# chanchanchan97/ICAFusion

Measured on AMD Instinct MI355X. Metric: RGB/IR image-pairs/sec (two-stream forward + NMS), higher is better.
Workload: dtype bf16

## Files before the change

### icafusion_amd/csrc/conv_common.h

```cpp
#pragma once
#include "icaf_common.h"

namespace icaf {

struct ConvP {
    const void* x; const void* w; const float* bias; void* y; const void* res;
    long long x_gs, w_gs, bias_gs, y_gs, res_gs;
    int B, H, W, Cin, ldx, Ho, Wo, Cout, ldy, kh, kw, sh, sw, ph, pw, ldr, Kp, act;
    int M, K, nchunks, mtiles, ntiles;
    int vec_y, vec_r;
    unsigned int x_bytes, w_bytes;
    float alpha_acc[2], alpha_res[2];
    const float* pre; int pre_h, pre_w, ldpre, pre_mode;
    const void* w1; const float* bias1;
    long long w1_gs, bias1_gs; int Kp1; unsigned int w1_bytes;
    const void* w2; const float* bias2; void* y2;
    long long w2_gs, bias2_gs, y2_gs; int Kp2, Cout2, ldy2, vec_y2, keep1; unsigned int w2_bytes;
    const void* x2; long long x2_gs; int ldx2;
};

constexpr int ROWB = 64;
constexpr int ROWS = 80;
constexpr int NTHREADS = 256;

int ctile_conv_check(const icaf_conv_args* a, const ConvP& p, int shape);
int launch_ctile(const icaf_conv_args* a, const ConvP& p, int shape, hipStream_t s);
const char* ctile_tag(int shape);
int stream_check(const icaf_conv_args* a, const ConvP& p, int shape);
int launch_stream(const icaf_conv_args* a, const ConvP& p, int shape, hipStream_t s);
const char* stream_tag(int shape);
int wreg_check(const icaf_conv_args* a, const ConvP& p, int shape);
int launch_wreg(const icaf_conv_args* a, const ConvP& p, int shape, hipStream_t s);
const char* wreg_tag(int shape);
int cstream_check(const icaf_conv_args* a, const ConvP& p, int shape);
int launch_cstream(const icaf_conv_args* a, const ConvP& p, int shape, hipStream_t s);
const char* cstream_tag(int shape);
int cwide_check(const icaf_conv_args* a, const ConvP& p, int shape);
int launch_cwide(const icaf_conv_args* a, const ConvP& p, int shape, hipStream_t s);
const char* cwide_tag(int shape);
int launch_bneck(const icaf_conv_args* a, const ConvP& p, int shape, hipStream_t s);

template <int ACT, int DT = ICAF_F32> __device__ __forceinline__ float apply_act(float v) {
    if constexpr (ACT == ICAF_ACT_SILU) return silu_f(v);
    else if constexpr (ACT == ICAF_ACT_GELU) return DT == ICAF_F32 ? gelu_f(v) : gelu_fast_f(v);
    else return v;
}
template <int ACT, int DT = ICAF_F32> __device__ __forceinline__ void apply_act4(const float (&x)[4], float (&y)[4]) {
    if constexpr (ACT == ICAF_ACT_SILU) silu4_f(x, y);
    else {
#pragma unroll
        for (int j = 0; j < 4; ++j) y[j] = apply_act<ACT, DT>(x[j]);
    }
}

__device__ __forceinline__ int xcd_tile(int ntile_total) {
    const int bid = blockIdx.x, q = ntile_total >> 3, r = ntile_total & 7, xcd = bid & 7, idx = bid >> 3;
    return (xcd < r ? xcd * (q + 1) : r * (q + 1) + (xcd - r) * q) + idx;
}

#ifndef ICAF_EPI_FAST
#define ICAF_EPI_FAST 1
#endif
#ifndef ICAF_PRE_WB
#define ICAF_PRE_WB 1
#endif
template <int DT, int ODT, int BM, int BN, int WM, int WN, int ACT, bool PRE, bool SECOND = false, bool WB = false, bool FULLVEC = false, typename RowMap>
__device__ __forceinline__ void epilogue(f32x16 (&acc)[WN / 32][WM / 32], unsigned char* lds, const ConvP& p, int g, RowMap row_to_m, int n0) {
    using E = Elem<DT>;
    using EO = Elem<ODT>;
    constexpr int TM = WM / 32, TN = WN / 32;
    constexpr int WAVES_M = BM / WM;
    constexpr int NT = (BM / WM) * (BN / WN) * 64;
    constexpr int VO = 16 / EO::BYTES;
    constexpr int SO = BN * EO::BYTES + 16;
    const int tid = threadIdx.x, lane = tid & 63, wave = tid >> 6, l31 = lane & 31, hi = lane >> 5;
    const int wm = wave % WAVES_M, wn = wave / WAVES_M;
    const float alpha_acc = SECOND ? 1.0f : p.alpha_acc[g], alpha_res = p.alpha_res[g];
    const float* __restrict__ bias = SECOND ? (p.bias2 ? p.bias2 + g * p.bias2_gs : nullptr) : (p.bias ? p.bias + g * p.bias_gs : nullptr);
    const int Cout = SECOND ? p.Cout2 : p.Cout, ldy = SECOND ? p.ldy2 : p.ldy, vec_y = SECOND ? p.vec_y2 : p.vec_y;
    if constexpr (PRE && ICAF_PRE_WB) {
        constexpr int SOF = BN * 4 + 16;
#pragma unroll
        for (int a = 0; a < TN; ++a) {
            f32x4 bq[4];
#pragma unroll
            for (int q = 0; q < 4; ++q) {
                const int n = n0 + wn * WN + a * 32 + 8 * q + 4 * hi;
                const bool okn = bias && n < Cout;
                const float* bp = okn ? bias + n : (const float*)p.w;
                const f32x4 t = *(const f32x4*)bp;
                bq[q] = okn ? t : f32x4{0.f, 0.f, 0.f, 0.f};
            }
#pragma unroll
            for (int q = 0; q < 4; ++q) {
                const int nl = wn * WN + a * 32 + 8 * q + 4 * hi;
#pragma unroll
                for (int b = 0; b < TM; ++b) {
                    const int ml = wm * WM + b * 32 + l31;
                    f32x4 t;
#pragma unroll
                    for (int j = 0; j < 4; ++j) t[j] = acc[a][b][4 * q + j] + bq[q][j];
                    *(f32x4*)(lds + ml * SOF + nl * 4) = t;
                }
            }
        }
        __syncthreads();
        typename EO::type* __restrict__ yg2 = SECOND ? (typename EO::type*)p.y2 + g * p.y2_gs : (typename EO::type*)p.y + g * p.y_gs;
        const typename E::type* __restrict__ rg2 = (!SECOND && p.res) ? (const typename E::type*)p.res + g * p.res_gs : nullptr;
        constexpr int VPR2 = BN / VO, NVEC2 = BM * VPR2, NIT2 = (NVEC2 + NT - 1) / NT;
        const float sy = (float)p.pre_h / (float)p.Ho, sx = (float)p.pre_w / (float)p.Wo;
#pragma unroll 2
        for (int it = 0; it < NIT2; ++it) {
            const int idx = tid + it * NT;
            if (idx >= NVEC2) break;
            const int row = idx / VPR2, cv = idx - row * VPR2;
            const int m = row_to_m(row), n = n0 + cv * VO;
            if (m < 0 || n >= Cout) continue;
            const float* pt4[4];
            float lx, ly;
            {
#pragma clang fp contract(off)
                const int wo = m % p.Wo, t = m / p.Wo, ho = t % p.Ho, bi = t / p.Ho;
                float fy = ((float)ho + 0.5f) * sy - 0.5f, fx = ((float)wo + 0.5f) * sx - 0.5f;
                fy = fy < 0.0f ? 0.0f : fy;
                fx = fx < 0.0f ? 0.0f : fx;
                int y0 = (int)fy, x0 = (int)fx;
                y0 = y0 < p.pre_h - 1 ? y0 : p.pre_h - 1;
                x0 = x0 < p.pre_w - 1 ? x0 : p.pre_w - 1;
                int y1 = y0 < p.pre_h - 1 ? y0 + 1 : y0, x1 = x0 < p.pre_w - 1 ? x0 + 1 : x0;
                ly = fy - (float)y0;
                lx = fx - (float)x0;
                if (p.pre_mode == 1) {
                    y0 = y1 = (int)((long long)ho * p.pre_h / p.Ho);
                    x0 = x1 = (int)((long long)wo * p.pre_w / p.Wo);
                    ly = lx = 0.0f;
                }
                const float* base = p.pre + (long long)bi * p.pre_h * p.pre_w * p.ldpre + n;
                pt4[0] = base + (long long)(y0 * p.pre_w + x0) * p.ldpre;
                pt4[1] = base + (long long)(y0 * p.pre_w + x1) * p.ldpre;
                pt4[2] = base + (long long)(y1 * p.pre_w + x0) * p.ldpre;
                pt4[3] = base + (long long)(y1 * p.pre_w + x1) * p.ldpre;
            }
            const int nvalid = (Cout - n) < VO ? (Cout - n) : VO;
            float v[VO];
#pragma unroll
            for (int k4 = 0; k4 < VO / 4; ++k4) {
                const f32x4 t = *(const f32x4*)(lds + row * SOF + (cv * VO + 4 * k4) * 4);
                float pv[4] = {0.f, 0.f, 0.f, 0.f};
                if (n + 4 * k4 < Cout) {
                    const f32x4 t00 = *(const f32x4*)(pt4[0] + 4 * k4), t01 = *(const f32x4*)(pt4[1] + 4 * k4);
                    const f32x4 t10 = *(const f32x4*)(pt4[2] + 4 * k4), t11 = *(const f32x4*)(pt4[3] + 4 * k4);
                    {
#pragma clang fp contract(off)
                        const float wx0 = 1.0f - lx, wy0 = 1.0f - ly;
#pragma unroll
                        for (int j = 0; j < 4; ++j) {
                            const float top = t00[j] * wx0 + t01[j] * lx;
                            const float bot = t10[j] * wx0 + t11[j] * lx;
                            pv[j] = top * wy0 + bot * ly;
                        }
                    }
                }
#pragma unroll
                for (int j = 0; j < 4; ++j) v[4 * k4 + j] = apply_act<ACT, DT>(t[j] + pv[j]) * alpha_acc;
            }
            u32x4 o = pack16<ODT>(v);
            typename EO::type* yp = yg2 + (long long)m * ldy + n;
            if (rg2) {
                unpack16<ODT>(o, v);
                const typename E::type* rp = rg2 + (long long)m * p.ldr + n;
                for (int j = 0; j < nvalid; ++j) v[j] = __builtin_fmaf(alpha_res, E::ld(rp + j), v[j]);
                o = pack16<ODT>(v);
            }
            if (vec_y && nvalid == VO) *(u32x4*)yp = o;
            else {
                unpack16<ODT>(o, v);
                for (int j = 0; j < nvalid; ++j) EO::st(yp + j, v[j]);
            }
        }
        return;
    }
    const float* pt[PRE ? TM : 1][4];
    float plx[PRE ? TM : 1], ply[PRE ? TM : 1];
    if constexpr (PRE) {
#pragma clang fp contract(off)
        const float sy = (float)p.pre_h / (float)p.Ho, sx = (float)p.pre_w / (float)p.Wo;
#pragma unroll
        for (int b = 0; b < TM; ++b) {
            const int m = row_to_m(wm * WM + b * 32 + l31);
            const int mm = m < 0 ? 0 : m;
            const int wo = mm % p.Wo, t = mm / p.Wo, ho = t % p.Ho, bi = t / p.Ho;
            float fy = ((float)ho + 0.5f) * sy - 0.5f, fx = ((float)wo + 0.5f) * sx - 0.5f;
            fy = fy < 0.0f ? 0.0f : fy;
            fx = fx < 0.0f ? 0.0f : fx;
            int y0 = (int)fy, x0 = (int)fx;
            y0 = y0 < p.pre_h - 1 ? y0 : p.pre_h - 1;
            x0 = x0 < p.pre_w - 1 ? x0 : p.pre_w - 1;
            int y1 = y0 < p.pre_h - 1 ? y0 + 1 : y0, x1 = x0 < p.pre_w - 1 ? x0 + 1 : x0;
            ply[b] = fy - (float)y0;
            plx[b] = fx - (float)x0;
            if (p.pre_mode == 1) {
                y0 = y1 = (int)((long long)ho * p.pre_h / p.Ho);
                x0 = x1 = (int)((long long)wo * p.pre_w / p.Wo);
                ply[b] = plx[b] = 0.0f;
            }
            const float* base = p.pre + (long long)bi * p.pre_h * p.pre_w * p.ldpre;
            pt[b][0] = base + (long long)(y0 * p.pre_w + x0) * p.ldpre;
            pt[b][1] = base + (long long)(y0 * p.pre_w + x1) * p.ldpre;
            pt[b][2] = base + (long long)(y1 * p.pre_w + x0) * p.ldpre;
            pt[b][3] = base + (long long)(y1 * p.pre_w + x1) * p.ldpre;
        }
    }
#pragma unroll
    for (int a = 0; a < TN; ++a) {
        f32x4 bq[4];
#pragma unroll
        for (int q = 0; q < 4; ++q) {
            const int n = n0 + wn * WN + a * 32 + 8 * q + 4 * hi;
            const bool okn = bias && n < Cout;
            const float* bp = okn ? bias + n : (const float*)p.w;
            const f32x4 t = *(const f32x4*)bp;
            bq[q] = okn ? t : f32x4{0.f, 0.f, 0.f, 0.f};
        }
#pragma unroll
        for (int q = 0; q < 4; ++q) {
            const int nl = wn * WN + a * 32 + 8 * q + 4 * hi;
            const float bv[4] = {bq[q][0], bq[q][1], bq[q][2], bq[q][3]};
#pragma unroll
            for (int b = 0; b < TM; ++b) {
                const int ml = wm * WM + b * 32 + l31;
                float pv[4] = {0.f, 0.f, 0.f, 0.f};
                if constexpr (PRE) if (n0 + nl < Cout) {
                    const f32x4 t00 = *(const f32x4*)(pt[b][0] + n0 + nl), t01 = *(const f32x4*)(pt[b][1] + n0 + nl);
                    const f32x4 t10 = *(const f32x4*)(pt[b][2] + n0 + nl), t11 = *(const f32x4*)(pt[b][3] + n0 + nl);
                    {
#pragma clang fp contract(off)
                        const float wx0 = 1.0f - plx[b], wy0 = 1.0f - ply[b];
#pragma unroll
                        for (int j = 0; j < 4; ++j) {
                            const float top = t00[j] * wx0 + t01[j] * plx[b];
                            const float bot = t10[j] * wx0 + t11[j] * plx[b];
                            pv[j] = top * wy0 + bot * ply[b];
                        }
                    }
                }
                float v[4], xin[4];
#pragma unroll
                for (int j = 0; j < 4; ++j) xin[j] = acc[a][b][4 * q + j] + bv[j] + pv[j];
                apply_act4<ACT, DT>(xin, v);
#pragma unroll
                for (int j = 0; j < 4; ++j) v[j] *= alpha_acc;
                unsigned char* dst = lds + ml * SO + nl * EO::BYTES;
                if constexpr (EO::BYTES == 4) {
                    *(f32x4*)dst = f32x4{v[0], v[1], v[2], v[3]};
                } else {
                    u32x2 pk;
                    if constexpr (ODT == ICAF_BF16) { pk[0] = pack2_bf16(v[0], v[1]); pk[1] = pack2_bf16(v[2], v[3]); }
                    else { pk[0] = pack2_f16(v[0], v[1]); pk[1] = pack2_f16(v[2], v[3]); }
                    *(u32x2*)dst = pk;
                }
            }
        }
    }
    __syncthreads();

    typename EO::type* __restrict__ yg = SECOND ? (typename EO::type*)p.y2 + g * p.y2_gs : (typename EO::type*)p.y + g * p.y_gs;
    const typename E::type* __restrict__ rg = (!SECOND && p.res) ? (const typename E::type*)p.res + g * p.res_gs : nullptr;
    constexpr int VPR = BN / VO;
    constexpr int NVEC = BM * VPR;
    constexpr int NIT = (NVEC + NT - 1) / NT;
    if constexpr (FULLVEC) {
        static_assert(!WB && NVEC % NT == 0 && (VPR & (VPR - 1)) == 0, "whole rounds of power-of-two rows");
#pragma unroll
        for (int it = 0; it < NIT; ++it) {
            const int idx = tid + it * NT, row = idx / VPR, cv = idx & (VPR - 1);
            const int m = row_to_m(row);
            if (m >= 0) *(u32x4*)(yg + (long long)m * ldy + n0 + cv * VO) = *(const u32x4*)(lds + row * SO + cv * 16);
        }
        return;
    }
#if ICAF_EPI_FAST
    if constexpr (VO == E::VEC && NVEC % NT == 0 && (VPR & (VPR - 1)) == 0) {
        if (vec_y && n0 + BN <= Cout && (!rg || p.vec_r)) {
            if (!rg) {
#pragma unroll
                for (int it = 0; it < NIT; ++it) {
                    const int idx = tid + it * NT, row = idx / VPR, cv = idx & (VPR - 1);
                    const int m = row_to_m(row);
                    if (m >= 0) *(u32x4*)(yg + (long long)m * ldy + n0 + cv * VO) = *(const u32x4*)(lds + row * SO + cv * 16);
                }
            } else {
                u32x4 rv[NIT];
#pragma unroll
                for (int it = 0; it < NIT; ++it) {
                    const int idx = tid + it * NT, row = idx / VPR, cv = idx & (VPR - 1);
                    const int m = row_to_m(row);
                    rv[it] = *(const u32x4*)(rg + (long long)(m < 0 ? 0 : m) * p.ldr + n0 + cv * VO);
                }
#pragma unroll
                for (int it = 0; it < NIT; ++it) {
                    const int idx = tid + it * NT, row = idx / VPR, cv = idx & (VPR - 1);
                    const int m = row_to_m(row);
                    if (m < 0) continue;
                    float v[VO], r[VO];
                    unpack16<ODT>(*(const u32x4*)(lds + row * SO + cv * 16), v);
                    unpack16<DT>(rv[it], r);
#pragma unroll
                    for (int j = 0; j < VO; ++j) v[j] = __builtin_fmaf(alpha_res, r[j], v[j]);
                    const u32x4 o = pack16<ODT>(v);
                    if constexpr (WB) *(u32x4*)(lds + row * SO + cv * 16) = o;
                    *(u32x4*)(yg + (long long)m * ldy + n0 + cv * VO) = o;
                }
            }
            return;
        }
#pragma unroll 1
        for (int it = 0; it < NIT; ++it) {
            const int idx = tid + it * NT, row = idx / VPR, cv = idx & (VPR - 1);
            const int m = row_to_m(row), n = n0 + cv * VO;
            if (m < 0 || n >= Cout) continue;
            const u32x4 sv = *(const u32x4*)(lds + row * SO + cv * 16);
// ... 141 lines not shown
```

### icafusion_amd/csrc/detect.hip

```cpp
#pragma clang fp contract(off)
#include "icaf_common.h"
#include "stream_core.h"
#include <cstdlib>

namespace icaf {

struct Anchors { float v[16]; };
int conv_prepare(const icaf_conv_args* a, ConvP& p);

struct DetectDiv { FastDiv no, nx, ny, na; };

template <bool I32>
__global__ __launch_bounds__(256) void detect_decode_kernel(const float* __restrict__ p, int ldp, float* __restrict__ z,
                                                            float* __restrict__ logits, float* __restrict__ raw, int B, int ny, int nx,
                                                            int na, int no, long long rows_total, long long row_offset, float stride,
                                                            Anchors anc, DetectDiv dv) {
    const long long total = (long long)B * na * ny * nx * no;
    for (long long e = (long long)blockIdx.x * blockDim.x + threadIdx.x; e < total; e += (long long)gridDim.x * blockDim.x) {
        int o, x, y, a, b;
        if constexpr (I32) {
            unsigned int q, r;
            fd_divmod((unsigned int)e, dv.no, q, r);
            o = (int)r;
            fd_divmod(q, dv.nx, q, r);
            x = (int)r;
            fd_divmod(q, dv.ny, q, r);
            y = (int)r;
            fd_divmod(q, dv.na, q, r);
            a = (int)r;
            b = (int)q;
        } else {
            o = (int)(e % no);
            const long long idx = e / no;
            x = (int)(idx % nx);
            long long t = idx / nx;
            y = (int)(t % ny);
            t /= ny;
            a = (int)(t % na);
            b = (int)(t / na);
        }
        const float v = p[(((long long)b * ny + y) * nx + x) * ldp + a * no + o];
        const long long row = (long long)b * rows_total + row_offset + ((long long)a * ny + y) * nx + x;
        if (raw) raw[e] = v;
        if (logits && o >= 5) logits[row * (no - 5) + (o - 5)] = v;
        const float sg = 1.0f / (1.0f + expf(-v));
        float out = sg;
        if (o == 0) out = ((sg * 2.0f - 0.5f) + (float)x) * stride;
        else if (o == 1) out = ((sg * 2.0f - 0.5f) + (float)y) * stride;
        else if (o == 2 || o == 3) {
            float an = anc.v[o - 2];
#pragma unroll
            for (int i = 1; i < 8; ++i) an = (a == i) ? (o == 2 ? anc.v[2 * i] : anc.v[2 * i + 1]) : an;
            const float d = sg * 2.0f;
            out = (d * d) * an;
        }
        z[row * no + o] = out;
    }
}

template <int NA, int NO>
__global__ __launch_bounds__(256) void detect_pixel_kernel(const float* __restrict__ p, int ldp, float* __restrict__ z,
                                                           float* __restrict__ logits, float* __restrict__ raw, int B, int ny, int nx,
                                                           long long rows_total, long long row_offset, float stride, Anchors anc,
                                                           FastDiv dnx, FastDiv dny) {
    constexpr int NV = NA * NO;
    const unsigned int total = (unsigned int)B * ny * nx;
    for (unsigned int pix = blockIdx.x * blockDim.x + threadIdx.x; pix < total; pix += gridDim.x * blockDim.x) {
        unsigned int t, x, b, y;
        fd_divmod(pix, dnx, t, x);
        fd_divmod(t, dny, b, y);
        const float* src = p + (long long)pix * ldp;
        float v[NV];
#pragma unroll
        for (int i = 0; i < NV; i += 2) {
            const float2 q = *(const float2*)(src + i);
            v[i] = q.x; v[i + 1] = q.y;
        }
#pragma unroll
        for (int a = 0; a < NA; ++a) {
            const long long cell = ((long long)a * ny + y) * nx + x;
            const long long row = (long long)b * rows_total + row_offset + cell;
            float o[NO];
#pragma unroll
            for (int k = 0; k < NO; ++k) {
                const float sg = 1.0f / (1.0f + expf(-v[a * NO + k]));
                float out = sg;
                if (k == 0) out = ((sg * 2.0f - 0.5f) + (float)x) * stride;
                else if (k == 1) out = ((sg * 2.0f - 0.5f) + (float)y) * stride;
                else if (k == 2 || k == 3) {
                    const float d = sg * 2.0f;
                    out = (d * d) * anc.v[2 * a + (k - 2)];
                }
                o[k] = out;
            }
            float* zr = z + row * NO;
#pragma unroll
            for (int k = 0; k < NO; k += 2) *(float2*)(zr + k) = float2{o[k], o[k + 1]};
            if (raw) {
                float* rr = raw + (((long long)b * NA) * ny * nx + cell) * NO;
#pragma unroll
                for (int k = 0; k < NO; k += 2) *(float2*)(rr + k) = float2{v[a * NO + k], v[a * NO + k + 1]};
            }
            if (logits) {
#pragma unroll
                for (int k = 5; k < NO; ++k) logits[row * (NO - 5) + (k - 5)] = v[a * NO + k];
            }
        }
    }
}

template <int NA, int NO>
static int launch_detect_pixel(const float* p, int ldp, float* z, float* logits, float* raw, int B, int ny, int nx, long long rows_total,
                               long long row_offset, float stride, const Anchors& anc, hipStream_t s) {
    const long long pixels = (long long)B * ny * nx;
    long long blocks = (pixels + 255) / 256;
    if (blocks > 256 * 32) blocks = 256 * 32;
    hipLaunchKernelGGL((detect_pixel_kernel<NA, NO>), dim3((unsigned)blocks), dim3(256), 0, s, p, ldp, z, logits, raw, B, ny, nx, rows_total,
                       row_offset, stride, anc, make_fastdiv((unsigned)nx), make_fastdiv((unsigned)ny));
    ICAF_LAUNCH_CHECK();
    return ICAF_OK;
}

template <int NA, int NO>
struct DetectEpi {
    static constexpr int SO = 64 * 4 + 16;
    float* z; float* logits; float* raw;
    int M, ny, nx; long long rows_total, row_offset; float stride; Anchors anc; FastDiv dnx, dny;
    template <int TM>
    __device__ __forceinline__ void stage(const f32x16 (&acc)[TM], const f32x4 (&bq)[4], unsigned char* stg, int row0, int col0, int l31, int hi, int, int) const {
#pragma unroll
        for (int qd = 0; qd < 4; ++qd) {
            const int nl = col0 + 8 * qd + 4 * hi;
#pragma unroll
            for (int b = 0; b < TM; ++b) {
                const int ml = row0 + b * 32 + l31;
                f32x4 v;
#pragma unroll
                for (int j = 0; j < 4; ++j) v[j] = acc[b][4 * qd + j] + bq[qd][j];
                *(f32x4*)(stg + ml * SO + nl * 4) = v;
            }
        }
    }
    __device__ __forceinline__ void flush(const unsigned char* stg, int m0, int n0, int tid) const {
        if (tid >= 128 * NA) return;
        const int row = tid / NA, a = tid - row * NA;
        const unsigned int pix = (unsigned int)(m0 + row);
        if ((int)pix >= M) return;
        unsigned int t, x, b, y;
        fd_divmod(pix, dnx, t, x);
        fd_divmod(t, dny, b, y);
        const float* src = (const float*)(stg + row * SO) + a * NO;
        float v[NO];
#pragma unroll
        for (int k = 0; k < NO; k += 2) { const float2 q2 = *(const float2*)(src + k); v[k] = q2.x; v[k + 1] = q2.y; }
        const long long cell = ((long long)a * ny + y) * nx + x;
        const long long zrow = (long long)b * rows_total + row_offset + cell;
        float o[NO];
#pragma unroll
        for (int k = 0; k < NO; ++k) {
            const float sg = 1.0f / (1.0f + expf(-v[k]));
            float out = sg;
            if (k == 0) out = ((sg * 2.0f - 0.5f) + (float)x) * stride;
            else if (k == 1) out = ((sg * 2.0f - 0.5f) + (float)y) * stride;
            else if (k == 2 || k == 3) {
                const float d = sg * 2.0f;
                out = (d * d) * anc.v[2 * a + (k - 2)];
            }
            o[k] = out;
        }
        float* zr = z + zrow * NO;
#pragma unroll
        for (int k = 0; k < NO; k += 2) *(float2*)(zr + k) = float2{o[k], o[k + 1]};
        if (raw) {
            float* rr = raw + (((long long)b * NA) * ny * nx + cell) * NO;
#pragma unroll
            for (int k = 0; k < NO; k += 2) *(float2*)(rr + k) = float2{v[k], v[k + 1]};
        }
        if (logits) {
#pragma unroll
            for (int k = 5; k < NO; ++k) logits[zrow * (NO - 5) + (k - 5)] = v[k];
        }
    }
};

template <int DT, int NA, int NO>
__global__ __launch_bounds__(512) void detect_conv_kernel(const ConvP p, const DetectEpi<NA, NO> epi) {
    stream_gemm<DT, 64, 1>(p, epi);
}

template <int DT, int NA, int NO>
static int launch_detect_conv(const ConvP& p, const DetectEpi<NA, NO>& epi, hipStream_t s) {
    constexpr int LDS = 3 * (128 + 64) * 128 + 128 * DetectEpi<NA, NO>::SO;
    ConvP q = p;
    q.mtiles = (p.M + 127) / 128;
    q.ntiles = 1;
    q.nchunks = p.K / 64;
    int dev = 0, cus = 256;
    ICAF_HIP(hipGetDevice(&dev));
    ICAF_HIP(hipDeviceGetAttribute(&cus, hipDeviceAttributeMultiprocessorCount, dev));
    const int grid = cus & ~7;
    ICAF_LDS_OPTIN((detect_conv_kernel<DT, NA, NO>), LDS);
    detect_conv_kernel<DT, NA, NO><<<dim3((unsigned)grid, 1, 1), dim3(512), LDS, s>>>(q, epi);
    ICAF_LAUNCH_CHECK();
    return ICAF_OK;
}

}

using namespace icaf;

enum { DETECT_PIXEL = 0, DETECT_ELEMENT = 1 };

static int detect_select(const float* p, int ldp, const float* z, const float* raw, int B, int ny, int nx, int na, int no) {
    const bool aligned = ldp % 2 == 0 && ((uintptr_t)p & 7) == 0 && ((uintptr_t)z & 7) == 0 && (!raw || ((uintptr_t)raw & 7) == 0);
    const bool pixel = na == 3 && (no == 6 || no == 8 || no == 14) && aligned && (long long)B * ny * nx < (1ll << 31) && !g_opt.detect_elementwise;
    return pixel ? DETECT_PIXEL : DETECT_ELEMENT;
}

extern "C" int icaf_detect_decode_kernel(const float* p, int ldp, const float* z, const float* raw, int B, int ny, int nx, int na, int no,
                                         int* kernel) {
    if (!p || !z || !kernel) return fail(ICAF_ERR_ARG, "icaf_detect_decode_kernel: null pointer");
    if (na < 1 || na > 8 || no < 6 || ldp < na * no) return fail(ICAF_ERR_ARG, "icaf_detect_decode_kernel: bad na/no/ldp");
    if (B < 1 || ny < 1 || nx < 1) return fail(ICAF_ERR_ARG, "icaf_detect_decode_kernel: empty level");
    *kernel = detect_select(p, ldp, z, raw, B, ny, nx, na, no);
    return ICAF_OK;
}

extern "C" int icaf_detect_decode(const float* p, int ldp, float* z, float* logits, float* raw, int B, int ny, int nx, int na, int no,
                                  long long rows_total, long long row_offset, float stride, const float* anchors_px, icaf_stream_t s) {
    if (!p || !z || !anchors_px) return fail(ICAF_ERR_ARG, "icaf_detect_decode: null pointer");
    if (na < 1 || na > 8 || no < 6 || ldp < na * no) return fail(ICAF_ERR_ARG, "icaf_detect_decode: bad na/no/ldp");
    if (row_offset + (long long)na * ny * nx > rows_total) return fail(ICAF_ERR_ARG, "icaf_detect_decode: level does not fit in z");
    Anchors anc;
    for (int i = 0; i < 16; ++i) anc.v[i] = i < 2 * na ? anchors_px[i] : 0.0f;
    const long long cells = (long long)B * na * ny * nx * no;
    long long blocks = (cells + 255) / 256;
    if (blocks > 256 * 32) blocks = 256 * 32;
    if (B < 1 || ny < 1 || nx < 1) return fail(ICAF_ERR_ARG, "icaf_detect_decode: empty level");
    if (detect_select(p, ldp, z, raw, B, ny, nx, na, no) == DETECT_PIXEL) {
        if (no == 6) return launch_detect_pixel<3, 6>(p, ldp, z, logits, raw, B, ny, nx, rows_total, row_offset, stride, anc, S(s));
        if (no == 8) return launch_detect_pixel<3, 8>(p, ldp, z, logits, raw, B, ny, nx, rows_total, row_offset, stride, anc, S(s));
        if (no == 14) return launch_detect_pixel<3, 14>(p, ldp, z, logits, raw, B, ny, nx, rows_total, row_offset, stride, anc, S(s));
    }
    const DetectDiv dv{make_fastdiv((unsigned)no), make_fastdiv((unsigned)nx), make_fastdiv((unsigned)ny), make_fastdiv((unsigned)na)};
    if (cells < (1ll << 31))
        hipLaunchKernelGGL(detect_decode_kernel<true>, dim3((unsigned)blocks), dim3(256), 0, S(s), p, ldp, z, logits, raw, B, ny, nx, na,
                           no, rows_total, row_offset, stride, anc, dv);
    else
        hipLaunchKernelGGL(detect_decode_kernel<false>, dim3((unsigned)blocks), dim3(256), 0, S(s), p, ldp, z, logits, raw, B, ny, nx, na,
                           no, rows_total, row_offset, stride, anc, dv);
    ICAF_LAUNCH_CHECK();
    return ICAF_OK;
}

extern "C" int icaf_detect_conv(const icaf_conv_args* a, float* z, float* logits, float* raw, int na, int no, long long rows_total,
                                long long row_offset, float stride, const float* anchors_px, icaf_stream_t s) {
    if (!a || !z || !anchors_px) return fail(ICAF_ERR_ARG, "icaf_detect_conv: null pointer");
    ConvP p;
    int st = conv_prepare(a, p);
    if (st) return st;
    if (a->dtype == ICAF_F32) return fail(ICAF_ERR_UNSUPPORTED, "icaf_detect_conv: 16-bit feature maps (the fp32 build runs icaf_conv2d + icaf_detect_decode)");
    if (a->kh != 1 || a->kw != 1 || a->sh != 1 || a->sw != 1 || a->ph || a->pw || a->groups != 1 || a->res || a->pre || a->w2 || a->act != ICAF_ACT_NONE)
        return fail(ICAF_ERR_ARG, "icaf_detect_conv: a plain 1x1 convolution without activation is expected");
    if ((a->Cin * 2) % 128 || p.x_bytes == 0) return fail(ICAF_ERR_UNSUPPORTED, "icaf_detect_conv: Cin * 2 bytes must be a multiple of 128 (Cin = %d)", a->Cin);
    if (na != 3 || (no != 6 && no != 8 && no != 14) || a->Cout != na * no) return fail(ICAF_ERR_UNSUPPORTED, "icaf_detect_conv: built for 3 anchors, no in {6, 8, 14} (na = %d, no = %d, Cout = %d)", na, no, a->Cout);
    if (row_offset + (long long)na * a->Ho * a->Wo > rows_total) return fail(ICAF_ERR_ARG, "icaf_detect_conv: level does not fit in z");
    if (((uintptr_t)z & 7) || (raw && ((uintptr_t)raw & 7))) return fail(ICAF_ERR_ARG, "icaf_detect_conv: z / raw must be 8-byte aligned");
    if ((long long)a->B * a->Ho * a->Wo >= (1ll << 31)) return fail(ICAF_ERR_UNSUPPORTED, "icaf_detect_conv: too many pixels");
    Anchors anc;
    for (int i = 0; i < 16; ++i) anc.v[i] = i < 2 * na ? anchors_px[i] : 0.0f;
    const FastDiv dnx = make_fastdiv((unsigned)a->Wo), dny = make_fastdiv((unsigned)a->Ho);
#define ICAF_DETECT_CONV(NO_)                                                                                                              \
    {                                                                                                                                      \
        DetectEpi<3, NO_> epi{z, logits, raw, p.M, a->Ho, a->Wo, rows_total, row_offset, stride, anc, dnx, dny};                           \
        return a->dtype == ICAF_BF16 ? launch_detect_conv<ICAF_BF16, 3, NO_>(p, epi, S(s)) : launch_detect_conv<ICAF_F16, 3, NO_>(p, epi, S(s)); \
    }
    if (no == 6) ICAF_DETECT_CONV(6)
    if (no == 8) ICAF_DETECT_CONV(8)
    ICAF_DETECT_CONV(14)
#undef ICAF_DETECT_CONV
}
```

### icafusion_amd/csrc/igemm_stream.hip

```cpp
#include "stream_core.h"

namespace icaf {

template <int DT, int BN, int ACT, bool PRE = false>
struct StoreEpi {
    using E = Elem<DT>;
    static constexpr int SO = BN * E::BYTES + 16;
    typename E::type* yg; float alpha_acc; int M, Cout, ldy;
    const typename E::type* rg; float alpha_res; int ldr;
    const float* pre; int pre_h, pre_w, ldpre, pre_mode, Ho, Wo;
    template <int TM>
    __device__ __forceinline__ void stage(const f32x16 (&acc)[TM], const f32x4 (&bq)[4], unsigned char* stg, int row0, int col0, int l31, int hi, int m0, int n0) const {
        const float* pt[PRE ? TM : 1][4];
        float plx[PRE ? TM : 1], ply[PRE ? TM : 1];
        if constexpr (PRE) {
#pragma clang fp contract(off)
            const float sy = (float)pre_h / (float)Ho, sx = (float)pre_w / (float)Wo;
#pragma unroll
            for (int b = 0; b < TM; ++b) {
                const int m = m0 + row0 + b * 32 + l31;
                const int mm = m < M ? m : 0;
                const int wo = mm % Wo, t = mm / Wo, ho = t % Ho, bi = t / Ho;
                float fy = ((float)ho + 0.5f) * sy - 0.5f, fx = ((float)wo + 0.5f) * sx - 0.5f;
                fy = fy < 0.0f ? 0.0f : fy;
                fx = fx < 0.0f ? 0.0f : fx;
                int y0 = (int)fy, x0 = (int)fx;
                y0 = y0 < pre_h - 1 ? y0 : pre_h - 1;
                x0 = x0 < pre_w - 1 ? x0 : pre_w - 1;
                int y1 = y0 < pre_h - 1 ? y0 + 1 : y0, x1 = x0 < pre_w - 1 ? x0 + 1 : x0;
                ply[b] = fy - (float)y0;
                plx[b] = fx - (float)x0;
                if (pre_mode == 1) {
                    y0 = y1 = (int)((long long)ho * pre_h / Ho);
                    x0 = x1 = (int)((long long)wo * pre_w / Wo);
                    ply[b] = plx[b] = 0.0f;
                }
                const float* base = pre + (long long)bi * pre_h * pre_w * ldpre;
                pt[b][0] = base + (long long)(y0 * pre_w + x0) * ldpre;
                pt[b][1] = base + (long long)(y0 * pre_w + x1) * ldpre;
                pt[b][2] = base + (long long)(y1 * pre_w + x0) * ldpre;
                pt[b][3] = base + (long long)(y1 * pre_w + x1) * ldpre;
            }
        }
#pragma unroll
        for (int qd = 0; qd < 4; ++qd) {
            const int nl = col0 + 8 * qd + 4 * hi;
#pragma unroll
            for (int b = 0; b < TM; ++b) {
                const int ml = row0 + b * 32 + l31;
                float pv[4] = {0.f, 0.f, 0.f, 0.f};
                if constexpr (PRE) if (n0 + nl < Cout) {
                    const f32x4 t00 = *(const f32x4*)(pt[b][0] + n0 + nl), t01 = *(const f32x4*)(pt[b][1] + n0 + nl);
                    const f32x4 t10 = *(const f32x4*)(pt[b][2] + n0 + nl), t11 = *(const f32x4*)(pt[b][3] + n0 + nl);
                    {
#pragma clang fp contract(off)
                        const float wx0 = 1.0f - plx[b], wy0 = 1.0f - ply[b];
#pragma unroll
                        for (int j = 0; j < 4; ++j) {
                            const float top = t00[j] * wx0 + t01[j] * plx[b];
                            const float bot = t10[j] * wx0 + t11[j] * plx[b];
                            pv[j] = top * wy0 + bot * ply[b];
                        }
                    }
                }
                float v[4];
#pragma unroll
                for (int j = 0; j < 4; ++j) v[j] = acc[b][4 * qd + j] + bq[qd][j] + pv[j];
                apply_act4<ACT, DT>(v, v);
#pragma unroll
                for (int j = 0; j < 4; ++j) v[j] *= alpha_acc;
                u32x2 pk;
                if constexpr (DT == ICAF_BF16) { pk[0] = pack2_bf16(v[0], v[1]); pk[1] = pack2_bf16(v[2], v[3]); }
                else { pk[0] = pack2_f16(v[0], v[1]); pk[1] = pack2_f16(v[2], v[3]); }
                *(u32x2*)(stg + ml * SO + nl * E::BYTES) = pk;
            }
        }
    }
    __device__ __forceinline__ void flush(const unsigned char* stg, int m0, int n0, int tid) const {
        constexpr int VPR = BN / E::VEC;
        constexpr int NIT = 128 * VPR / 512;
#pragma unroll
        for (int itv = 0; itv < NIT; ++itv) {
            const int idx = tid + itv * 512;
            const int row = idx / VPR, cv = idx - row * VPR;
            const int m = m0 + row, n = n0 + cv * E::VEC;
            u32x4 sv = *(const u32x4*)(stg + row * SO + cv * 16);
            if (m < M && n < Cout) {
                if (rg) {
                    float v[E::VEC], r[E::VEC];
                    unpack16<DT>(sv, v);
                    unpack16<DT>(*(const u32x4*)(rg + (long long)m * ldr + n), r);
#pragma unroll
                    for (int j = 0; j < E::VEC; ++j) v[j] = __builtin_fmaf(alpha_res, r[j], v[j]);
                    sv = pack16<DT>(v);
                }
                *(u32x4*)(yg + (long long)m * ldy + n) = sv;
            }
        }
    }
};

template <int DT, int BN, int ACT, int MODE, bool PRE = false>
__global__ __launch_bounds__(512) void igemm_stream_kernel(const ConvP p) {
    using E = Elem<DT>;
    const int g = blockIdx.z;
    const StoreEpi<DT, BN, ACT, PRE> epi{(typename E::type*)p.y + g * p.y_gs, p.alpha_acc[g], p.M, p.Cout, p.ldy,
                                         p.res ? (const typename E::type*)p.res + g * p.res_gs : nullptr, p.alpha_res[g], p.ldr,
                                         p.pre, p.pre_h, p.pre_w, p.ldpre, p.pre_mode, p.Ho, p.Wo};
    stream_gemm<DT, BN, MODE>(p, epi);
}

const char* stream_tag(int shape) { return shape == 1 ? "128x128" : shape == 2 ? "128x64" : "?"; }

static int stream_grid(int groups, int* wgx) {
    int dev = 0, cus = 256;
    ICAF_HIP(hipGetDevice(&dev));
    ICAF_HIP(hipDeviceGetAttribute(&cus, hipDeviceAttributeMultiprocessorCount, dev));
    *wgx = ((cus / (groups > 0 ? groups : 1)) & ~7) >> 3;
    return ICAF_OK;
}

int stream_check(const icaf_conv_args* a, const ConvP& p, int shape) {
    if (shape < 1 || shape > 2) return fail(ICAF_ERR_ARG, "igemm_stream: unknown shape %d", shape);
    if (a->dtype == ICAF_F32 || a->out_dtype != a->dtype) return fail(ICAF_ERR_UNSUPPORTED, "igemm_stream: 16-bit types, out dtype == dtype");
    if ((a->Cin * 2) % 128) return fail(ICAF_ERR_UNSUPPORTED, "igemm_stream: Cin * 2 bytes must be a multiple of 128 (Cin = %d)", a->Cin);
    if (a->w2) return fail(ICAF_ERR_UNSUPPORTED, "igemm_stream: no chained layer");
    if (a->pre && (a->act != ICAF_ACT_SILU || a->kh != 1 || a->kw != 1 || a->sh != 1 || a->sw != 1 || a->ph || a->pw || a->groups != 1))
        return fail(ICAF_ERR_UNSUPPORTED, "igemm_stream: the pre-activation term is built for 1x1 SiLU layers (one group)");
    if (a->res && !p.vec_r) return fail(ICAF_ERR_UNSUPPORTED, "igemm_stream: the residual must take 16-byte vectors");
    if (p.x_bytes == 0) return fail(ICAF_ERR_UNSUPPORTED, "igemm_stream: operand exceeds the 2 GiB buffer-descriptor range");
    if (!p.vec_y || a->Cout % 8) return fail(ICAF_ERR_UNSUPPORTED, "igemm_stream: y must take 16-byte vectors (ldy %% 8, Cout %% 8, alignment)");
    if (shape == 1 && a->Cout <= 64) return fail(ICAF_ERR_UNSUPPORTED, "igemm_stream 128x128: Cout = %d <= 64 (use 128x64)", a->Cout);
    int wgx = 0;
    const int st = stream_grid(a->groups, &wgx);
    if (st) return st;
    const int ntiles = (p.Cout + (shape == 1 ? 128 : 64) - 1) / (shape == 1 ? 128 : 64);
    if (wgx < ntiles || wgx % ntiles) return fail(ICAF_ERR_UNSUPPORTED, "igemm_stream: %d channel tiles do not divide the %d workgroups of an XCD", ntiles, wgx);
    return ICAF_OK;
}

template <int DT, int BN, int ACT>
static int launch_stream_cfg(const ConvP& p, int groups, hipStream_t s) {
    constexpr int LDS = 3 * (128 + BN) * 128 + 128 * (BN * 2 + 16);
    ConvP q = p;
    q.mtiles = (p.M + 127) / 128;
    q.ntiles = (p.Cout + BN - 1) / BN;
    q.nchunks = p.K / 64;
    int dev = 0, wgx = 0;
    ICAF_HIP(hipGetDevice(&dev));
    if (dev < 0 || dev >= ICAF_MAX_DEVICES) return fail(ICAF_ERR_UNSUPPORTED, "device ordinal %d", dev);
    int st = stream_grid(groups, &wgx);
    if (st) return st;
    const int grid = wgx << 3;
    if (wgx < q.ntiles || wgx % q.ntiles) return fail(ICAF_ERR_UNSUPPORTED, "igemm_stream: %d channel tiles do not divide the %d workgroups of an XCD", q.ntiles, wgx);
    const bool plain = q.kh == 1 && q.kw == 1 && q.sh == 1 && q.sw == 1 && q.ph == 0 && q.pw == 0;
    auto go = [&](auto kern) -> int {
        ICAF_LDS_OPTIN(kern, LDS);
        kern<<<dim3((unsigned)grid, 1, (unsigned)groups), dim3(512), LDS, s>>>(q);
        ICAF_LAUNCH_CHECK();
        return ICAF_OK;
    };
    if constexpr (ACT == ICAF_ACT_SILU) { if (p.pre) return go(igemm_stream_kernel<DT, BN, ACT, 1, true>); }
    if (plain) return go(igemm_stream_kernel<DT, BN, ACT, 1>);
    return go(igemm_stream_kernel<DT, BN, ACT, 2>);
}

template <int DT, int BN>
static int launch_stream_act(const ConvP& p, int groups, hipStream_t s) {
    if (p.act == ICAF_ACT_SILU) return launch_stream_cfg<DT, BN, ICAF_ACT_SILU>(p, groups, s);
    if (p.act == ICAF_ACT_GELU) return launch_stream_cfg<DT, BN, ICAF_ACT_GELU>(p, groups, s);
    return launch_stream_cfg<DT, BN, ICAF_ACT_NONE>(p, groups, s);
}

int launch_stream(const icaf_conv_args* a, const ConvP& p, int shape, hipStream_t s) {
    if (a->dtype == ICAF_BF16) return shape == 1 ? launch_stream_act<ICAF_BF16, 128>(p, a->groups, s) : launch_stream_act<ICAF_BF16, 64>(p, a->groups, s);
    return shape == 1 ? launch_stream_act<ICAF_F16, 128>(p, a->groups, s) : launch_stream_act<ICAF_F16, 64>(p, a->groups, s);
}

}
```

### icafusion_amd/csrc/stream_core.h

```cpp
#pragma once
#include "conv_common.h"

namespace icaf {

template <int DT, int BN, int MODE, class EPI>
__device__ __forceinline__ void stream_gemm(const ConvP& p, const EPI& epi) {
    using E = Elem<DT>;
    static_assert(DT != ICAF_F32, "16-bit types");
    constexpr int BM = 128, RB = 128, NS = 3, NW = 8;
    constexpr int WN = 32, WM = BN == 128 ? 64 : 32;
    constexpr int TM = WM / 32, TN = 1;
    constexpr int WAVES_M = BM / WM;
    constexpr int VEC = E::VEC;
    constexpr int RPI = 8;
    constexpr int NA = BM / RPI / NW, NB = BN / RPI / NW;
    constexpr int PER = NA + NB;
    constexpr int STAGE = (BM + BN) * RB;
    constexpr int NSTEP = RB / 32;
    constexpr int RING = NS * STAGE;
    static_assert(NA >= 1 && NB >= 1 && (BN == 128 || BN == 64), "tile shape");
    extern __shared__ __attribute__((aligned(1024))) unsigned char lds[];
    unsigned char* stg = lds + RING;

    const int tid = threadIdx.x, lane = tid & 63, l31 = lane & 31, hi = lane >> 5;
    const int wave = __builtin_amdgcn_readfirstlane(tid >> 6);
    const int g = blockIdx.z;
    const int wm = wave % WAVES_M, wn = wave / WAVES_M;

    const __amdgpu_buffer_rsrc_t xr = __builtin_amdgcn_make_buffer_rsrc(
        (void*)((const typename E::type*)p.x + g * p.x_gs), 0, p.x_bytes, 0x00020000);
    const __amdgpu_buffer_rsrc_t wr = __builtin_amdgcn_make_buffer_rsrc(
        (void*)((const typename E::type*)p.w + g * p.w_gs), 0, p.w_bytes, 0x00020000);
    constexpr unsigned OOB = 0x80000000u;

    const int rsub = lane >> 3;
    const int dkey = ((wave & 1) << 2) | (rsub >> 1);
    const int lslot = (lane & 7) ^ dkey;

    const int xcd = blockIdx.x & 7, lb = blockIdx.x >> 3, wgx = gridDim.x >> 3;
    const int per_xcd = (p.mtiles + 7) >> 3, m_lo = xcd * per_xcd, m_hi = min(m_lo + per_xcd, p.mtiles);
    const int nt = lb % p.ntiles, mstride = wgx / p.ntiles, m_first = m_lo + lb / p.ntiles;
    const int n0 = nt * BN;
    const int nch = p.nchunks;

    int it = m_first, ic = 0;
    int kc = 0, ky = 0, kx = 0;
    unsigned ia_off[NA], iw_off[NB];
    int ia_h0[NA], ia_w0[NA];
#pragma unroll
    for (int i = 0; i < NB; ++i)
        iw_off[i] = ((unsigned)(n0 + (wave + NW * i) * RPI + rsub) * (unsigned)p.Kp + (unsigned)(lslot * VEC)) * E::BYTES;
    auto issue_setup = [&]() {
        const bool live = it < m_hi;
#pragma unroll
        for (int i = 0; i < NA; ++i) {
            const int m = it * BM + (wave + NW * i) * RPI + rsub;
            const bool ok = live && m < p.M;
            if constexpr (MODE == 1) {
                ia_off[i] = ok ? ((unsigned)m * (unsigned)p.ldx + (unsigned)(lslot * VEC)) * E::BYTES : OOB;
            } else {
                const int mm = ok ? m : 0;
                const int wo = mm % p.Wo, t = mm / p.Wo, ho = t % p.Ho, b = t / p.Ho;
                ia_h0[i] = ok ? ho * p.sh - p.ph : -0x10000;
                ia_w0[i] = wo * p.sw - p.pw;
                ia_off[i] = (unsigned)b * (unsigned)(p.H * p.W) * (unsigned)p.ldx * (unsigned)E::BYTES
                          + (unsigned)((ia_h0[i] * p.W + ia_w0[i]) * p.ldx + lslot * VEC) * E::BYTES;
            }
        }
    };
    auto issue_part = [&](int stage, int part) {
        unsigned char* st = lds + stage * STAGE;
        const unsigned koff = (unsigned)ic * RB;
        unsigned tap_delta = 0;
        if constexpr (MODE == 2) tap_delta = (unsigned)((ky * p.W + kx) * p.ldx + kc) * E::BYTES;
#pragma unroll
        for (int i = 0; i < NA; ++i) {
            if (i % NSTEP != part) continue;
            unsigned voff;
            if constexpr (MODE == 1) {
                voff = ia_off[i] == OOB ? OOB : ia_off[i] + koff;
            } else {
                const int h = ia_h0[i] + ky, w = ia_w0[i] + kx;
                const bool ok = (unsigned)h < (unsigned)p.H && (unsigned)w < (unsigned)p.W;
                voff = ok ? ia_off[i] + tap_delta : OOB;
            }
            __builtin_amdgcn_raw_ptr_buffer_load_lds(xr, (lds_ptr_t)(st + (wave + NW * i) * 1024), 16, voff, 0, 0, 0);
        }
#pragma unroll
        for (int i = 0; i < NB; ++i) {
            if ((NA + i) % NSTEP != part) continue;
            const unsigned voff = it < m_hi ? iw_off[i] + koff : OOB;
            __builtin_amdgcn_raw_ptr_buffer_load_lds(wr, (lds_ptr_t)(st + BM * RB + (wave + NW * i) * 1024), 16, voff, 0, 0, 0);
        }
    };
    auto issue_advance = [&]() {
        if constexpr (MODE == 2) {
            kc += RB / E::BYTES;
            if (kc >= p.Cin) { kc = 0; if (++kx == p.kw) { kx = 0; ++ky; } }
        }
        if (++ic == nch) {
            ic = 0; kc = 0; ky = 0; kx = 0;
            it += mstride;
            issue_setup();
        }
    };

    const float* __restrict__ bias = p.bias ? p.bias + g * p.bias_gs : nullptr;
    f32x4 bq[4];
#pragma unroll
    for (int qd = 0; qd < 4; ++qd) {
        const int n = n0 + wn * WN + 8 * qd + 4 * hi;
        const bool okn = bias && n < p.Cout;
        const float* bp = okn ? bias + n : (const float*)p.w;
        const f32x4 t = *(const f32x4*)bp;
        bq[qd] = okn ? t : f32x4{0.f, 0.f, 0.f, 0.f};
    }
#pragma unroll
    for (int qd = 0; qd < 4; ++qd) asm volatile("" : "+v"(bq[qd]));

    if (m_first >= m_hi) return;

    const int fkey = (l31 >> 1) & 7;
    int foff[NSTEP];
#pragma unroll
    for (int s = 0; s < NSTEP; ++s) foff[s] = l31 * RB + (((2 * s + hi) ^ fkey) << 4);

    issue_setup();
#pragma unroll
    for (int s = 0; s < NS; ++s) {
#pragma unroll
        for (int part = 0; part < NSTEP; ++part) issue_part(s, part);
        issue_advance();
    }

    int q = 0;
    for (int mt = m_first; mt < m_hi; mt += mstride) {
        const int m0 = mt * BM;
        f32x16 acc[TM];
#pragma unroll
        for (int b = 0; b < TM; ++b)
#pragma unroll
            for (int r = 0; r < 16; ++r) acc[b][r] = 0.0f;
        for (int c = 0; c < nch; ++c, ++q) {
            wait_vmcnt<PER>();
            asm volatile("s_waitcnt lgkmcnt(0)" ::: "memory");
            __builtin_amdgcn_s_barrier();
            const int sq = q % NS;
            const unsigned char* a_s = lds + sq * STAGE;
            const unsigned char* b_s = a_s + BM * RB;
            u32x4 fp[NSTEP][TM], fw[NSTEP];
#pragma unroll
            for (int s = 0; s < NSTEP; ++s) {
#pragma unroll
                for (int b = 0; b < TM; ++b) fp[s][b] = *(const u32x4*)(a_s + (wm * WM + b * 32) * RB + foff[s]);
                fw[s] = *(const u32x4*)(b_s + (wn * WN) * RB + foff[s]);
            }
            const int sfree = (q + NS - 1) % NS;
#pragma unroll
            for (int s = 0; s < NSTEP; ++s) {
#pragma unroll
                for (int b = 0; b < TM; ++b) mma_step<DT>(acc[b], fw[s], fp[s][b]);
                if (q > 0) issue_part(sfree, s);
            }
            if (q > 0) issue_advance();
        }

        epi.stage(acc, bq, stg, wm * WM, wn * WN, l31, hi, m0, n0);
        lds_barrier();
        epi.flush(stg, m0, n0, tid);
    }
    wait_vmcnt<0>();
}


}
```

Measured before the change: 17200.

## Restructure PRE-fused SiLU epilogue to gather bilinear taps per output vector

Adds a specialized epilogue for the prefix-upsample-add path. It stages fp32 accumulators through LDS in halves, and each thread loads its bilinear taps for the contiguous 8-channel vector it stores, with the tap loads for the next half issued early. Division by Wo/Ho uses precomputed fast divisors. The aim is coalesced, vectorized tap gathers instead of the per-fragment scattered 4-wide loads done inside the MFMA layout. In exchange it adds extra barriers and register pressure from prefetched taps, and staging fp32 changes the LDS footprint.

```diff
diff --git a/icafusion_amd/csrc/conv_common.h b/icafusion_amd/csrc/conv_common.h
--- a/icafusion_amd/csrc/conv_common.h
+++ b/icafusion_amd/csrc/conv_common.h
@@ -17,6 +17,7 @@
     const void* w2; const float* bias2; void* y2;
     long long w2_gs, bias2_gs, y2_gs; int Kp2, Cout2, ldy2, vec_y2, keep1; unsigned int w2_bytes;
     const void* x2; long long x2_gs; int ldx2;
+    FastDiv fd_wo, fd_ho;
 };
 
 constexpr int ROWB = 64;
diff --git a/icafusion_amd/csrc/detect.hip b/icafusion_amd/csrc/detect.hip
--- a/icafusion_amd/csrc/detect.hip
+++ b/icafusion_amd/csrc/detect.hip
@@ -123,6 +123,7 @@
 
 template <int NA, int NO>
 struct DetectEpi {
+    static constexpr bool OWNS_TILE = false;
     static constexpr int SO = 64 * 4 + 16;
     float* z; float* logits; float* raw;
     int M, ny, nx; long long rows_total, row_offset; float stride; Anchors anc; FastDiv dnx, dny;
diff --git a/icafusion_amd/csrc/igemm_stream.hip b/icafusion_amd/csrc/igemm_stream.hip
--- a/icafusion_amd/csrc/igemm_stream.hip
+++ b/icafusion_amd/csrc/igemm_stream.hip
@@ -5,64 +5,20 @@
 template <int DT, int BN, int ACT, bool PRE = false>
 struct StoreEpi {
     using E = Elem<DT>;
-    static constexpr int SO = BN * E::BYTES + 16;
+    static constexpr bool OWNS_TILE = false;
+    static constexpr int SO = BN * E::BYTES + 16, STG_BYTES = 128 * SO;
     typename E::type* yg; float alpha_acc; int M, Cout, ldy;
     const typename E::type* rg; float alpha_res; int ldr;
-    const float* pre; int pre_h, pre_w, ldpre, pre_mode, Ho, Wo;
+    const float* pre; int pre_h, pre_w, ldpre, pre_mode, Ho, Wo; FastDiv fd_wo, fd_ho;
     template <int TM>
-    __device__ __forceinline__ void stage(const f32x16 (&acc)[TM], const f32x4 (&bq)[4], unsigned char* stg, int row0, int col0, int l31, int hi, int m0, int n0) const {
-        const float* pt[PRE ? TM : 1][4];
-        float plx[PRE ? TM : 1], ply[PRE ? TM : 1];
-        if constexpr (PRE) {
-#pragma clang fp contract(off)
-            const float sy = (float)pre_h / (float)Ho, sx = (float)pre_w / (float)Wo;
-#pragma unroll
-            for (int b = 0; b < TM; ++b) {
-                const int m = m0 + row0 + b * 32 + l31;
-                const int mm = m < M ? m : 0;
-                const int wo = mm % Wo, t = mm / Wo, ho = t % Ho, bi = t / Ho;
-                float fy = ((float)ho + 0.5f) * sy - 0.5f, fx = ((float)wo + 0.5f) * sx - 0.5f;
-                fy = fy < 0.0f ? 0.0f : fy;
-                fx = fx < 0.0f ? 0.0f : fx;
-                int y0 = (int)fy, x0 = (int)fx;
-                y0 = y0 < pre_h - 1 ? y0 : pre_h - 1;
-                x0 = x0 < pre_w - 1 ? x0 : pre_w - 1;
-                int y1 = y0 < pre_h - 1 ? y0 + 1 : y0, x1 = x0 < pre_w - 1 ? x0 + 1 : x0;
-                ply[b] = fy - (float)y0;
-                plx[b] = fx - (float)x0;
-                if (pre_mode == 1) {
-                    y0 = y1 = (int)((long long)ho * pre_h / Ho);
-                    x0 = x1 = (int)((long long)wo * pre_w / Wo);
-                    ply[b] = plx[b] = 0.0f;
-                }
-                const float* base = pre + (long long)bi * pre_h * pre_w * ldpre;
-                pt[b][0] = base + (long long)(y0 * pre_w + x0) * ldpre;
-                pt[b][1] = base + (long long)(y0 * pre_w + x1) * ldpre;
-                pt[b][2] = base + (long long)(y1 * pre_w + x0) * ldpre;
-                pt[b][3] = base + (long long)(y1 * pre_w + x1) * ldpre;
-            }
-        }
+    __device__ __forceinline__ void stage(const f32x16 (&acc)[TM], const f32x4 (&bq)[4], unsigned char* stg, int row0, int col0, int l31, int hi, int, int) const {
 #pragma unroll
         for (int qd = 0; qd < 4; ++qd) {
             const int nl = col0 + 8 * qd + 4 * hi;
 #pragma unroll
             for (int b = 0; b < TM; ++b) {
                 const int ml = row0 + b * 32 + l31;
-                float pv[4] = {0.f, 0.f, 0.f, 0.f};
-                if constexpr (PRE) if (n0 + nl < Cout) {
-                    const f32x4 t00 = *(const f32x4*)(pt[b][0] + n0 + nl), t01 = *(const f32x4*)(pt[b][1] + n0 + nl);
-                    const f32x4 t10 = *(const f32x4*)(pt[b][2] + n0 + nl), t11 = *(const f32x4*)(pt[b][3] + n0 + nl);
-                    {
-#pragma clang fp contract(off)
-                        const float wx0 = 1.0f - plx[b], wy0 = 1.0f - ply[b];
-#pragma unroll
-                        for (int j = 0; j < 4; ++j) {
-                            const float top = t00[j] * wx0 + t01[j] * plx[b];
-                            const float bot = t10[j] * wx0 + t11[j] * plx[b];
-                            pv[j] = top * wy0 + bot * ply[b];
-                        }
-                    }
-                }
+                const float pv[4] = {0.f, 0.f, 0.f, 0.f};
                 float v[4];
 #pragma unroll
                 for (int j = 0; j < 4; ++j) v[j] = acc[b][4 * qd + j] + bq[qd][j] + pv[j];
@@ -100,13 +56,153 @@
     }
 };
 
+template <int DT, int BN, int ACT>
+struct StoreEpi<DT, BN, ACT, true> {
+    using E = Elem<DT>;
+    static constexpr bool OWNS_TILE = true;
+    static constexpr int NH = BN / 64;
+    static constexpr int SO = BN * 4 + 16, STG_BYTES = 128 / NH * SO;
+    static constexpr int VPR = BN / E::VEC;
+    static constexpr int NIT = 128 / NH * VPR / 512;
+    typename E::type* yg; float alpha_acc; int M, Cout, ldy;
+    const typename E::type* rg; float alpha_res; int ldr;
+    const float* pre; int pre_h, pre_w, ldpre, pre_mode, Ho, Wo;
+    FastDiv fd_wo, fd_ho;
+    struct Taps { f32x4 t[NIT][4][2]; float lx[NIT], ly[NIT]; };
+
+    static __device__ __forceinline__ void vec_of(int idx, int h, int& lr, int& cv, int& row) {
+        lr = idx / VPR;
+        cv = idx - lr * VPR;
+        row = (lr >> 5) * (32 * NH) + h * 32 + (lr & 31);
+    }
+
+    template <bool FULL>
+    __device__ __forceinline__ void load_taps(Taps& tp, int m0, int n0, int tid, int h) const {
+#pragma clang fp contract(off)
+        const float sy = (float)pre_h / (float)Ho, sx = (float)pre_w / (float)Wo;
+#pragma unroll
+        for (int itv = 0; itv < NIT; ++itv) {
+            int lr, cv, row;
+            vec_of(tid + itv * 512, h, lr, cv, row);
+            const int m = m0 + row, n = n0 + cv * E::VEC;
+            const bool ok = FULL || (m < M && n < Cout);
+            const int mm = ok ? m : 0, nn = ok ? n : 0;
+            unsigned t, uwo, ubi, uho;
+            fd_divmod((unsigned)mm, fd_wo, t, uwo);
+            fd_divmod(t, fd_ho, ubi, uho);
+            const int wo = (int)uwo, ho = (int)uho, bi = (int)ubi;
+            float fy = ((float)ho + 0.5f) * sy - 0.5f, fx = ((float)wo + 0.5f) * sx - 0.5f;
+            fy = fy < 0.0f ? 0.0f : fy;
+            fx = fx < 0.0f ? 0.0f : fx;
+            int y0 = (int)fy, x0 = (int)fx;
+            y0 = y0 < pre_h - 1 ? y0 : pre_h - 1;
+            x0 = x0 < pre_w - 1 ? x0 : pre_w - 1;
+            int y1 = y0 < pre_h - 1 ? y0 + 1 : y0, x1 = x0 < pre_w - 1 ? x0 + 1 : x0;
+            tp.ly[itv] = fy - (float)y0;
+            tp.lx[itv] = fx - (float)x0;
+            if (pre_mode == 1) {
+                y0 = y1 = (int)((long long)ho * pre_h / Ho);
+                x0 = x1 = (int)((long long)wo * pre_w / Wo);
+                tp.ly[itv] = tp.lx[itv] = 0.0f;
+            }
+            const float* base = pre + (long long)bi * pre_h * pre_w * ldpre + nn;
+            const float* pt[4] = {base + (long long)(y0 * pre_w + x0) * ldpre, base + (long long)(y0 * pre_w + x1) * ldpre,
+                                  base + (long long)(y1 * pre_w + x0) * ldpre, base + (long long)(y1 * pre_w + x1) * ldpre};
+#pragma unroll
+            for (int k = 0; k < 4; ++k) {
+                tp.t[itv][k][0] = *(const f32x4*)pt[k];
+                tp.t[itv][k][1] = *(const f32x4*)(pt[k] + 4);
+            }
+        }
+    }
+
+    template <int TM>
+    __device__ __forceinline__ void tile(const f32x16 (&acc)[TM], const f32x4 (&bq)[4], unsigned char* stg, int row0, int col0, int l31, int hi,
+                                         int m0, int n0, int tid) const {
+        if (m0 + 128 <= M && n0 + BN <= Cout) tile_body<true>(acc, bq, stg, row0, col0, l31, hi, m0, n0, tid);
+        else tile_body<false>(acc, bq, stg, row0, col0, l31, hi, m0, n0, tid);
+    }
+    template <bool FULL, int TM>
+    __device__ __forceinline__ void tile_body(const f32x16 (&acc)[TM], const f32x4 (&bq)[4], unsigned char* stg, int row0, int col0, int l31, int hi,
+                                              int m0, int n0, int tid) const {
+        static_assert(TM == NH, "one accumulator block per pass");
+        const int ls = row0 / (32 * TM) * 32 + l31;
+        Taps tp;
+        load_taps<FULL>(tp, m0, n0, tid, 0);
+#pragma unroll
+        for (int h = 0; h < NH; ++h) {
+            if (h) lds_barrier();
+#pragma unroll
+            for (int qd = 0; qd < 4; ++qd) {
+                f32x4 t;
+#pragma unroll
+                for (int j = 0; j < 4; ++j) t[j] = acc[h][4 * qd + j] + bq[qd][j];
+                *(f32x4*)(stg + ls * SO + (col0 + 8 * qd + 4 * hi) * 4) = t;
+            }
+            lds_barrier();
+            u32x4 out[NIT];
+#pragma unroll
+            for (int itv = 0; itv < NIT; ++itv) {
+                int lr, cv, row;
+                vec_of(tid + itv * 512, h, lr, cv, row);
+                float v[E::VEC];
+#pragma unroll
+                for (int k4 = 0; k4 < 2; ++k4) {
+                    const f32x4 s = *(const f32x4*)(stg + lr * SO + (cv * E::VEC + 4 * k4) * 4);
+                    const f32x4 t00 = tp.t[itv][0][k4], t01 = tp.t[itv][1][k4], t10 = tp.t[itv][2][k4], t11 = tp.t[itv][3][k4];
+                    float x[4], a[4];
+                    {
+#pragma clang fp contract(off)
+                        const float lx = tp.lx[itv], ly = tp.ly[itv], wx0 = 1.0f - lx, wy0 = 1.0f - ly;
+#pragma unroll
+                        for (int j = 0; j < 4; ++j) {
+                            const float top = t00[j] * wx0 + t01[j] * lx;
+                            const float bot = t10[j] * wx0 + t11[j] * lx;
+                            const float pv = top * wy0 + bot * ly;
+                            x[j] = s[j] + pv;
+                        }
+                    }
+                    apply_act4<ACT, DT>(x, a);
+#pragma unroll
+                    for (int j = 0; j < 4; ++j) v[4 * k4 + j] = a[j] * alpha_acc;
+                }
+                out[itv] = pack16<DT>(v);
+            }
+            if (rg) {
+#pragma unroll
+                for (int itv = 0; itv < NIT; ++itv) {
+                    int lr, cv, row;
+                    vec_of(tid + itv * 512, h, lr, cv, row);
+                    const int m = m0 + row, n = n0 + cv * E::VEC;
+                    if (FULL || (m < M && n < Cout)) {
+                        float v[E::VEC], r[E::VEC];
+                        unpack16<DT>(out[itv], v);
+                        unpack16<DT>(*(const u32x4*)(rg + (long long)m * ldr + n), r);
+#pragma unroll
+                        for (int j = 0; j < E::VEC; ++j) v[j] = __builtin_fmaf(alpha_res, r[j], v[j]);
+                        out[itv] = pack16<DT>(v);
+                    }
+                }
+            }
+            if (h + 1 < NH) load_taps<FULL>(tp, m0, n0, tid, h + 1);
+#pragma unroll
+            for (int itv = 0; itv < NIT; ++itv) {
+                int lr, cv, row;
+                vec_of(tid + itv * 512, h, lr, cv, row);
+                const int m = m0 + row, n = n0 + cv * E::VEC;
+                if (FULL || (m < M && n < Cout)) *(u32x4*)(yg + (long long)m * ldy + n) = out[itv];
+            }
+        }
+    }
+};
+
 template <int DT, int BN, int ACT, int MODE, bool PRE = false>
 __global__ __launch_bounds__(512) void igemm_stream_kernel(const ConvP p) {
     using E = Elem<DT>;
     const int g = blockIdx.z;
     const StoreEpi<DT, BN, ACT, PRE> epi{(typename E::type*)p.y + g * p.y_gs, p.alpha_acc[g], p.M, p.Cout, p.ldy,
                                          p.res ? (const typename E::type*)p.res + g * p.res_gs : nullptr, p.alpha_res[g], p.ldr,
-                                         p.pre, p.pre_h, p.pre_w, p.ldpre, p.pre_mode, p.Ho, p.Wo};
+                                         p.pre, p.pre_h, p.pre_w, p.ldpre, p.pre_mode, p.Ho, p.Wo, p.fd_wo, p.fd_ho};
     stream_gemm<DT, BN, MODE>(p, epi);
 }
 
@@ -141,7 +237,7 @@
 
 template <int DT, int BN, int ACT>
 static int launch_stream_cfg(const ConvP& p, int groups, hipStream_t s) {
-    constexpr int LDS = 3 * (128 + BN) * 128 + 128 * (BN * 2 + 16);
+    constexpr int RING = 3 * (128 + BN) * 128;
     ConvP q = p;
     q.mtiles = (p.M + 127) / 128;
     q.ntiles = (p.Cout + BN - 1) / BN;
@@ -154,15 +250,17 @@
     const int grid = wgx << 3;
     if (wgx < q.ntiles || wgx % q.ntiles) return fail(ICAF_ERR_UNSUPPORTED, "igemm_stream: %d channel tiles do not divide the %d workgroups of an XCD", q.ntiles, wgx);
     const bool plain = q.kh == 1 && q.kw == 1 && q.sh == 1 && q.sw == 1 && q.ph == 0 && q.pw == 0;
-    auto go = [&](auto kern) -> int {
-        ICAF_LDS_OPTIN(kern, LDS);
-        kern<<<dim3((unsigned)grid, 1, (unsigned)groups), dim3(512), LDS, s>>>(q);
+    auto go = [&](auto kern, int lds) -> int {
+        ICAF_LDS_OPTIN(kern, lds);
+        kern<<<dim3((unsigned)grid, 1, (unsigned)groups), dim3(512), lds, s>>>(q);
         ICAF_LAUNCH_CHECK();
         return ICAF_OK;
     };
-    if constexpr (ACT == ICAF_ACT_SILU) { if (p.pre) return go(igemm_stream_kernel<DT, BN, ACT, 1, true>); }
-    if (plain) return go(igemm_stream_kernel<DT, BN, ACT, 1>);
-    return go(igemm_stream_kernel<DT, BN, ACT, 2>);
+    q.fd_wo = make_fastdiv((unsigned)p.Wo);
+    q.fd_ho = make_fastdiv((unsigned)p.Ho);
+    if constexpr (ACT == ICAF_ACT_SILU) { if (p.pre) return go(igemm_stream_kernel<DT, BN, ACT, 1, true>, RING + StoreEpi<DT, BN, ACT, true>::STG_BYTES); }
+    if (plain) return go(igemm_stream_kernel<DT, BN, ACT, 1>, RING + StoreEpi<DT, BN, ACT>::STG_BYTES);
+    return go(igemm_stream_kernel<DT, BN, ACT, 2>, RING + StoreEpi<DT, BN, ACT>::STG_BYTES);
 }
 
 template <int DT, int BN>
diff --git a/icafusion_amd/csrc/stream_core.h b/icafusion_amd/csrc/stream_core.h
--- a/icafusion_amd/csrc/stream_core.h
+++ b/icafusion_amd/csrc/stream_core.h
@@ -165,9 +165,13 @@
             if (q > 0) issue_advance();
         }
 
-        epi.stage(acc, bq, stg, wm * WM, wn * WN, l31, hi, m0, n0);
-        lds_barrier();
-        epi.flush(stg, m0, n0, tid);
+        if constexpr (EPI::OWNS_TILE) {
+            epi.tile(acc, bq, stg, wm * WM, wn * WN, l31, hi, m0, n0, tid);
+        } else {
+            epi.stage(acc, bq, stg, wm * WM, wn * WN, l31, hi, m0, n0);
+            lds_barrier();
+            epi.flush(stg, m0, n0, tid);
+        }
     }
     wait_vmcnt<0>();
 }
```

After: 17190. Within noise of the previous version (-0.0%).
